# cvxpy/cvxpylayers

Measured on NVIDIA H100. Metric: QP problems/sec fwd+bwd (batch=4096, n=100, m=200, zero+nonneg cones), higher is better.
Workload: dtype f64

## Files before the change

cvxpylayers_b200/csrc/common.cuh:

```cuda
#pragma once
#include <cuda_runtime.h>
#include <stdint.h>
#include <stddef.h>
#include "../../include/bcone.h"

#define BC_TAU_FACTOR 10.0
#define BC_ZERO_CONE_FACTOR 1000.0
#define BC_MIN_SCALE 1e-4
#define BC_MAX_SCALE 1e4
#define BC_RESCALE_MIN_ITERS 100
#define BC_EQ_MIN 1e-4
#define BC_EQ_MAX 1e4

enum { BC_CZERO = 0, BC_CNONNEG = 1, BC_CSOC = 2, BC_CPSD = 3 };

struct DevStruct {
  int n, m, nnzA, nnzP;
  int z, l, nq, ns;
  int ep, ed, exp_start;
  int dense;
  int ncones;
  int max_psd;
  const int *A_indptr, *A_indices;
  const int *At_colptr, *At_rowidx, *At_perm;
// ... 384 lines not shown
__device__ __forceinline__ void dmma884(double &d0, double &d1, double a, double b) {
  asm volatile("mma.sync.aligned.m8n8k4.row.col.f64.f64.f64.f64 {%0,%1}, {%2}, {%3}, {%0,%1};" : "+d"(d0), "+d"(d1) : "d"(a), "d"(b));
}

__device__ __forceinline__ double c_mul_sub(double c, double x, double s, double y) { return fma(c, x, -(s * y)); }
__device__ __forceinline__ double c_mul_add(double s, double x, double c, double y) { return fma(s, x, c * y); }

template <bool SQ = false, class Layout, class Epi>
__device__ __forceinline__ void matvec_rows(const double *__restrict__ M, Layout lay, int nrows, int ncols,
                                            const double *x, Epi ep) {
  const int lane = threadIdx.x & 31, warp = threadIdx.x >> 5, nw = blockDim.x >> 5;
  if (ncols <= 128) {
    double xr[4];
#pragma unroll
    for (int k = 0; k < 4; k++) { const int c = lane + 32 * k; xr[k] = c < ncols ? x[c] : 0.0; }
    for (int i0 = warp * 4; i0 < nrows; i0 += nw * 4) {
      int o[4], b[4], e[4];
#pragma unroll
      for (int r = 0; r < 4; r++) {
        const int i = i0 + r; const bool ok = i < nrows;
        o[r] = ok ? lay.base(i) : 0; b[r] = ok ? lay.beg(i) : 0; e[r] = ok ? lay.end(i) : 0;
      }
      double a[4] = {0, 0, 0, 0};
#pragma unroll
      for (int k = 0; k < 4; k++) {
        const int c = lane + 32 * k;
#pragma unroll
        for (int r = 0; r < 4; r++)
          if (c >= b[r] && c < e[r]) { const double q = M[o[r] + c]; a[r] = fma(SQ ? q * q : q, xr[k], a[r]); }
      }
      const double k = butterfly4(a[0], a[1], a[2], a[3], lane);
      if ((lane & 7) == 0) {
        const int r = i0 + ((lane >> 4) & 1) * 2 + ((lane >> 3) & 1);
        if (r < nrows) ep(r, k);
      }
    }
  } else {
    for (int i0 = warp * 4; i0 < nrows; i0 += nw * 4) {
      int o[4], b[4], e[4];
      int lmax = 0, bmin = 1 << 30;
#pragma unroll
      for (int r = 0; r < 4; r++) {
        const int i = i0 + r; const bool ok = i < nrows;
        o[r] = ok ? lay.base(i) : 0; b[r] = ok ? lay.beg(i) : 0; e[r] = ok ? lay.end(i) : 0;
        lmax = max(lmax, e[r]); if (ok) bmin = min(bmin, b[r]);
      }
      double a[4] = {0, 0, 0, 0};
      for (int c = (min(bmin, lmax) & ~31) + lane; c < lmax; c += 32) {
        const double xv = x[c];
#pragma unroll
        for (int r = 0; r < 4; r++)
          if (c >= b[r] && c < e[r]) { const double q = M[o[r] + c]; a[r] = fma(SQ ? q * q : q, xv, a[r]); }
      }
      const double k = butterfly4(a[0], a[1], a[2], a[3], lane);
      if ((lane & 7) == 0) {
        const int r = i0 + ((lane >> 4) & 1) * 2 + ((lane >> 3) & 1);
        if (r < nrows) ep(r, k);
      }
    }
  }
}

struct ColPlan {
  int j, lo, hi, CH;
  bool active, fits;
};
__device__ __forceinline__ ColPlan make_colplan(int nrows, int ncols) {
  ColPlan p;
  const int T = blockDim.x, t = threadIdx.x;
  p.fits = ncols <= T;
  p.CH = p.fits ? T / ncols : 1;
  p.j = p.fits ? t % ncols : t;
  const int c = p.fits ? t / ncols : 0;
  p.active = p.fits && c < p.CH;
  p.lo = (c * nrows) / p.CH;
  p.hi = ((c + 1) * nrows) / p.CH;
  return p;
}

template <bool SQ = false, class Layout, class Epi>
__device__ __forceinline__ void matvec_cols(const double *__restrict__ M, Layout lay, int nrows, int ncols,
                                            const double *y, double *part, Epi ep, const ColPlan &pl) {
  const int T = blockDim.x, t = threadIdx.x;
  if (pl.fits) {
    if (pl.active) {
      const int j = pl.j;
      int i = max(pl.lo, lay.row_lo(j));
      const int hi = min(pl.hi, lay.row_hi(j, nrows));
      double a0 = 0, a1 = 0;
      if (i < hi) {
        const double *p = M + lay.base(i) + j;
        if (Layout::kFullRows) {
          const int st = lay.step(0);
          for (; i + 3 < hi; i += 4) {
            const double q0 = p[0], q1 = p[st], q2 = p[2 * st], q3 = p[3 * st];
            a0 = fma(SQ ? q0 * q0 : q0, y[i], a0); a1 = fma(SQ ? q1 * q1 : q1, y[i + 1], a1);
            a0 = fma(SQ ? q2 * q2 : q2, y[i + 2], a0); a1 = fma(SQ ? q3 * q3 : q3, y[i + 3], a1);
            p += 4 * st;
          }
          for (; i < hi; i++) { const double q = p[0]; a0 = fma(SQ ? q * q : q, y[i], a0); p += st; }
        } else {
          for (; i + 1 < hi; i += 2) {
            const int s0 = lay.step(i);
            const double q0 = p[0], q1 = p[s0];
            a0 = fma(SQ ? q0 * q0 : q0, y[i], a0); a1 = fma(SQ ? q1 * q1 : q1, y[i + 1], a1);
            p += s0 + lay.step(i + 1);
          }
          if (i < hi) { const double q = p[0]; a0 = fma(SQ ? q * q : q, y[i], a0); }
        }
      }
      part[t] = a0 + a1;
    }
    __syncthreads();
    if (t < ncols) {
      double a = 0;
      for (int cc = 0; cc < pl.CH; cc++) a += part[cc * ncols + t];
      ep(t, a);
    }
    __syncthreads();
  } else {
    for (int j = t; j < ncols; j += T) {
      double a = 0;
      const int hi = lay.row_hi(j, nrows);
      for (int i = lay.row_lo(j); i < hi; i++) { const double q = M[lay.base(i) + j]; a = fma(SQ ? q * q : q, y[i], a); }
      ep(j, a);
    }
    __syncthreads();
  }
}

template <bool SQ = false, class Epi>
__device__ __forceinline__ void dense_rows2(const double *__restrict__ A, int m, int n, const double *x, Epi ep) {
  const int lane = threadIdx.x & 31, warp = threadIdx.x >> 5, nw = blockDim.x >> 5;
  const bool ok0 = 2 * lane < n, ok1 = 2 * lane + 64 < n;
  const double2 x0 = ok0 ? make_double2(x[2 * lane], x[2 * lane + 1]) : make_double2(0.0, 0.0);
  const double2 x1 = ok1 ? make_double2(x[2 * lane + 64], x[2 * lane + 65]) : make_double2(0.0, 0.0);
  for (int i0 = warp * 4; i0 < m; i0 += nw * 4) {
    double a[4] = {0, 0, 0, 0};
#pragma unroll
    for (int r = 0; r < 4; r++) {
      const int i = i0 + r;
      if (i < m) {
        const double2 *p2 = reinterpret_cast<const double2 *>(A + i * n) + lane;
        if (ok0) { double2 q = p2[0]; if (SQ) { q.x *= q.x; q.y *= q.y; } a[r] = fma(q.x, x0.x, a[r]); a[r] = fma(q.y, x0.y, a[r]); }
        if (ok1) { double2 q = p2[32]; if (SQ) { q.x *= q.x; q.y *= q.y; } a[r] = fma(q.x, x1.x, a[r]); a[r] = fma(q.y, x1.y, a[r]); }
      }
    }
    const double tot = butterfly4(a[0], a[1], a[2], a[3], lane);
    if ((lane & 7) == 0) {
      const int i = i0 + ((lane >> 4) & 1) * 2 + ((lane >> 3) & 1);
      if (i < m) ep(i, tot);
    }
  }
}
template <bool SQ = false, class Epi>
__device__ __forceinline__ void dense_cols2(const double *__restrict__ A, int m, int n, const double *y, double *part, Epi ep) {
  const int T = blockDim.x, t = threadIdx.x, npair = n >> 1;
  const int CH = min(8, T / npair), pr = t % npair, c = t / npair;
  if (c < CH) {
    const int lo = (c * m) / CH, hi = ((c + 1) * m) / CH;
    const double2 *p2 = reinterpret_cast<const double2 *>(A + lo * n) + pr;
    double2 a0 = make_double2(0.0, 0.0), a1 = make_double2(0.0, 0.0);
    int i = lo;
    for (; i + 1 < hi; i += 2) {
      double2 q0 = p2[0], q1 = p2[npair];
      if (SQ) { q0.x *= q0.x; q0.y *= q0.y; q1.x *= q1.x; q1.y *= q1.y; }
      const double y0 = y[i], y1 = y[i + 1];
      a0.x = fma(q0.x, y0, a0.x); a0.y = fma(q0.y, y0, a0.y);
      a1.x = fma(q1.x, y1, a1.x); a1.y = fma(q1.y, y1, a1.y);
      p2 += 2 * npair;
    }
    if (i < hi) { double2 q0 = p2[0]; if (SQ) { q0.x *= q0.x; q0.y *= q0.y; } const double y0 = y[i]; a0.x = fma(q0.x, y0, a0.x); a0.y = fma(q0.y, y0, a0.y); }
    *reinterpret_cast<double2 *>(part + c * n + 2 * pr) = make_double2(a0.x + a1.x, a0.y + a1.y);
  }
  __syncthreads();
  if (t < n) {
    double a = 0;
    for (int cc = 0; cc < CH; cc++) a += part[cc * n + t];
    ep(t, a);
  }
  __syncthreads();
}

template <bool SQ = false, class Epi>
__device__ __forceinline__ void csr_rows(const double *__restrict__ vals, const int *__restrict__ indptr,
                                         const int *__restrict__ indices, int nrows,
                                         const double *x, Epi ep) {
  constexpr int G = 4;
  const int g = threadIdx.x % G, grp = threadIdx.x / G, ngrp = blockDim.x / G;
  for (int base = 0; base < nrows; base += ngrp) {
    const int i = base + grp;
    double a = 0;
    if (i < nrows) {
      const int e = __ldg(indptr + i + 1);
      for (int k = __ldg(indptr + i) + g; k < e; k += G) { const double q = vals[k]; a = fma(SQ ? q * q : q, x[__ldg(indices + k)], a); }
    }
    a += __shfl_xor_sync(0xffffffffu, a, 1);
    a += __shfl_xor_sync(0xffffffffu, a, 2);
    if (g == 0 && i < nrows) ep(i, a);
  }
}
template <bool SQ = false, class Epi>
__device__ __forceinline__ void csr_cols(const double *__restrict__ vals, const int *__restrict__ colptr,
                                         const int *__restrict__ rowidx, const int *__restrict__ perm, int ncols,
                                         const double *y, Epi ep) {
  constexpr int G = 4;
  const int g = threadIdx.x % G, grp = threadIdx.x / G, ngrp = blockDim.x / G;
  for (int base = 0; base < ncols; base += ngrp) {
    const int j = base + grp;
    double a = 0;
    if (j < ncols) {
      const int e = __ldg(colptr + j + 1);
      for (int k = __ldg(colptr + j) + g; k < e; k += G) { const double q = vals[__ldg(perm + k)]; a = fma(SQ ? q * q : q, y[__ldg(rowidx + k)], a); }
    }
    a += __shfl_xor_sync(0xffffffffu, a, 1);
    a += __shfl_xor_sync(0xffffffffu, a, 2);
    if (g == 0 && j < ncols) ep(j, a);
  }
}

template <bool DENSE, bool SQ = false, class Epi>
__device__ __forceinline__ void A_mul(const DevStruct &S, const double *Av, const double *x, Epi ep, bool wide = false) {
  if (DENSE && wide) dense_rows2<SQ>(Av, S.m, S.n, x, ep);
  else if (DENSE) matvec_rows<SQ>(Av, DenseLayout{S.n}, S.m, S.n, x, ep);
  else csr_rows<SQ>(Av, S.A_indptr, S.A_indices, S.m, x, ep);
}
template <bool DENSE, bool SQ = false, class Epi>
__device__ __forceinline__ void AT_mul(const DevStruct &S, const double *Av, const double *y, double *part, Epi ep, const ColPlan &plA,
                                       bool wide = false) {
  if (DENSE && wide) dense_cols2<SQ>(Av, S.m, S.n, y, part, ep);
  else if (DENSE) matvec_cols<SQ>(Av, DenseLayout{S.n}, S.m, S.n, y, part, ep, plA);
  else { csr_cols<SQ>(Av, S.At_colptr, S.At_rowidx, S.At_perm, S.n, y, ep); __syncthreads(); }
}

template <bool SQ = false, class Epi>
__device__ __forceinline__ void P_mul(const DevStruct &S, const double *Pv, const double *x, double *part, Epi ep, const ColPlan &plN) {
  const int n = S.n;
  if (S.p_dense) {
    matvec_rows<SQ>(Pv, PackedUpperLayout<false>{n}, n, n, x, ep);
    __syncthreads();
    matvec_cols<SQ>(Pv, PackedUpperLayout<true>{n}, n, n, x, part, ep, plN);
  } else {
    csr_rows<SQ>(Pv, S.P_indptr, S.P_indices, n, x, ep);
    __syncthreads();
    constexpr int G = 4;
    const int g = threadIdx.x % G, grp = threadIdx.x / G, ngrp = blockDim.x / G;
    for (int base = 0; base < n; base += ngrp) {
      const int j = base + grp;
      double a = 0;
      if (j < n) {
        const int e = __ldg(S.Pt_colptr + j + 1);
        for (int k = __ldg(S.Pt_colptr + j) + g; k < e; k += G) {
          const int i = __ldg(S.Pt_rowidx + k);
          if (i != j) { const double q = Pv[__ldg(S.Pt_perm + k)]; a = fma(SQ ? q * q : q, x[i], a); }
        }
      }
      a += __shfl_xor_sync(0xffffffffu, a, 1);
      a += __shfl_xor_sync(0xffffffffu, a, 2);
      if (g == 0 && j < n) ep(j, a);
    }
    __syncthreads();
  }
}

__host__ __device__ __forceinline__ int chol_held_cols(int threads) { return 8 * (threads > 32 ? (threads >> 5) - 1 : 1); }
__host__ __device__ __forceinline__ int chol_scratch_doubles(int n, int threads) {
  const int ld = 8 * ((n + 7) >> 3) - chol_held_cols(threads);
  return 8 * (ld > 0 ? ld : 0) + 2;
}
__device__ __forceinline__ double rsqrt_nr(double x) {
  double y;
  asm("rsqrt.approx.ftz.f64 %0, %1;" : "=d"(y) : "d"(x));
  double e = fma(-x * y, y, 1.0);
  y = fma(0.5 * y, e, y);
  e = fma(-x * y, y, 1.0);
  return fma(0.5 * y, e, y);
}
struct Tri4 { double l00, l10, l11, l20, l21, l22, l30, l31, l32, l33, m00, m10, m11, m20, m21, m22, m30, m31, m32, m33; bool pd; };
__device__ __forceinline__ Tri4 tri4_block(const double *K, int r0, int jb) {
  Tri4 q;
  const double *R0 = K + ((r0 * (r0 + 1)) >> 1) + r0;
  const double *R1 = K + (((r0 + 1) * (r0 + 2)) >> 1) + r0, *R2 = K + (((r0 + 2) * (r0 + 3)) >> 1) + r0, *R3 = K + (((r0 + 3) * (r0 + 4)) >> 1) + r0;
  const double d00 = R0[0];
  const double d10 = jb > 1 ? R1[0] : 0.0, d11 = jb > 1 ? R1[1] : 1.0;
  const double d20 = jb > 2 ? R2[0] : 0.0, d21 = jb > 2 ? R2[1] : 0.0, d22 = jb > 2 ? R2[2] : 1.0;
  const double d30 = jb > 3 ? R3[0] : 0.0, d31 = jb > 3 ? R3[1] : 0.0, d32 = jb > 3 ? R3[2] : 0.0, d33 = jb > 3 ? R3[3] : 1.0;
  const double p0 = d00, r0_ = rsqrt_nr(p0);
  q.l00 = p0 * r0_; q.l10 = d10 * r0_; q.l20 = d20 * r0_; q.l30 = d30 * r0_;
  const double p1 = fma(-q.l10, q.l10, d11), r1_ = rsqrt_nr(p1);
  q.l11 = p1 * r1_; q.l21 = fma(-q.l20, q.l10, d21) * r1_; q.l31 = fma(-q.l30, q.l10, d31) * r1_;
  const double p2 = fma(-q.l21, q.l21, fma(-q.l20, q.l20, d22)), r2_ = rsqrt_nr(p2);
  q.l22 = p2 * r2_; q.l32 = fma(-q.l31, q.l21, fma(-q.l30, q.l20, d32)) * r2_;
  const double p3 = fma(-q.l32, q.l32, fma(-q.l31, q.l31, fma(-q.l30, q.l30, d33))), r3_ = rsqrt_nr(p3);
  q.l33 = p3 * r3_;
  q.pd = (p0 > 0) && (p1 > 0) && (p2 > 0) && (p3 > 0);
  q.m00 = r0_; q.m11 = r1_; q.m22 = r2_; q.m33 = r3_;
  q.m10 = -q.l10 * q.m00 * r1_;
  q.m20 = -fma(q.l21, q.m10, q.l20 * q.m00) * r2_; q.m21 = -q.l21 * q.m11 * r2_;
  q.m30 = -fma(q.l32, q.m20, fma(q.l31, q.m10, q.l30 * q.m00)) * r3_;
  q.m31 = -fma(q.l32, q.m21, q.l31 * q.m11) * r3_; q.m32 = -q.l32 * q.m22 * r3_;
  return q;
}
#ifdef BC_CHOLPROF
#define CP_STAMP(k) if (prof && t == 0) { const long long now_ = clock64(); atomicAdd(prof + (k), (unsigned long long)(now_ - tt)); tt = now_; }
#else
#define CP_STAMP(k)
#endif
static __device__ __noinline__ bool chol_inv_packed(double *K, int n, double *tmp, unsigned long long *prof = nullptr) {
  const int T = blockDim.x, t = threadIdx.x, lane = t & 31, warp = t >> 5, nw = T >> 5;
  const int W = nw > 1 ? nw - 1 : 1, w0 = nw > 1 ? warp - 1 : 0, held = chol_held_cols(T);
  const int lds = max(0, 8 * ((n + 7) >> 3) - held);
  double *Tst = tmp, *flag = tmp + 8 * lds;
  double h0 = 0.0, h1 = 0.0;
  long long t0 = 0;
  if (prof && t == 0) t0 = clock64();
#ifdef BC_CHOLPROF
  long long tt = t0;
#endif
  const int fr = lane >> 2, fc = lane & 3;
  auto rowp = [&](int i) { return K + ((i * (i + 1)) >> 1); };
  auto put_m = [&](int r0, int jb, const Tri4 &q) {
    double *D0 = rowp(r0) + r0;
    D0[0] = q.m00;
    if (jb > 1) { double *D1 = rowp(r0 + 1) + r0; D1[0] = q.m10; D1[1] = q.m11; }
    if (jb > 2) { double *D2 = rowp(r0 + 2) + r0; D2[0] = q.m20; D2[1] = q.m21; D2[2] = q.m22; }
    if (jb > 3) { double *D3 = rowp(r0 + 3) + r0; D3[0] = q.m30; D3[1] = q.m31; D3[2] = q.m32; D3[3] = q.m33; }
  };
  auto diag_block = [&](int J0) {
    const int jb = min(8, n - J0), jb2 = jb - 4;
    const Tri4 a = tri4_block(K, J0, min(4, jb));
    bool pd = a.pd;
    __syncwarp();
    if (lane == 0) put_m(J0, min(4, jb), a);
    if (jb2 > 0) {
      const int r = fr, c = fc;
      const bool own = lane < 16 && r < jb2;
      double *Rr = rowp(J0 + 4 + r) + J0;
      __syncwarp();
      double v = 0.0;
      if (own) {
#pragma unroll
        for (int k = 0; k < 4; k++)
          if (k <= c) v = fma(Rr[k], rowp(J0 + c)[J0 + k], v);
      }
      __syncwarp();
      if (own) Rr[c] = v;
      __syncwarp();
      if (own && c <= r) {
        const double *Rc = rowp(J0 + 4 + c) + J0;
        double g = Rr[4 + c];
#pragma unroll
        for (int k = 0; k < 4; k++) g = fma(-Rr[k], Rc[k], g);
        Rr[4 + c] = g;
      }
      __syncwarp();
      const Tri4 b = tri4_block(K, J0 + 4, jb2);
      pd = pd && b.pd;
      double u = 0.0;
      if (own) {
#pragma unroll
        for (int k = 0; k < 4; k++)
          if (k >= c) u = fma(Rr[k], rowp(J0 + k)[J0 + c], u);
      }
      __syncwarp();
      if (lane == 0) put_m(J0 + 4, jb2, b);
      __syncwarp();
      double s = 0.0;
#pragma unroll
      for (int k = 0; k < 4; k++) {
        const double uk = __shfl_sync(0xffffffffu, u, 4 * k + c);
        if (own && k <= r) s = fma(Rr[4 + k], uk, s);
      }
      if (own) Rr[c] = -s;
    }
    if (lane == 0 && !pd) *flag = 0.0;
  };
  auto trail_tile = [&](int ta, int tb, int J0, int jb, int R0) {
    const int ra = R0 + 8 * ta + fr, rb = R0 + 8 * tb + fr;
    const double *La = rowp(ra) + J0, *Lb = rowp(rb) + J0;
    const double fa0 = (ra < n && fc < jb) ? -La[fc] : 0.0, fa1 = (ra < n && fc + 4 < jb) ? -La[fc + 4] : 0.0;
    const double fb0 = (rb < n && fc < jb) ? Lb[fc] : 0.0, fb1 = (rb < n && fc + 4 < jb) ? Lb[fc + 4] : 0.0;
    const int cc = R0 + 8 * tb + 2 * fc;
    double *pc = rowp(ra) + cc;
    const bool ok0 = ra < n && cc <= ra, ok1 = ra < n && cc + 1 <= ra;
    double c0 = ok0 ? pc[0] : 0.0, c1 = ok1 ? pc[1] : 0.0;
    dmma884(c0, c1, fa0, fb0);
    dmma884(c0, c1, fa1, fb1);
    if (ok0) pc[0] = c0;
    if (ok1) pc[1] = c1;
  };
  auto inv_tile = [&](int jt, int I0, int ib) {
    double c0 = 0.0, c1 = 0.0, d0 = 0.0, d1 = 0.0;
    const bool zr = fr < ib;
    const double *zrow = rowp(I0 + (zr ? fr : 0));
    const int jcol = 8 * jt + fr;
    int k0 = 8 * jt + fc;
    {
      const double a0 = zr ? zrow[k0] : 0.0, a1 = zr ? zrow[k0 + 4] : 0.0;
      const double b0 = jcol <= k0 ? rowp(k0)[jcol] : 0.0, b1 = jcol <= k0 + 4 ? rowp(k0 + 4)[jcol] : 0.0;
      dmma884(c0, c1, a0, b0);
      dmma884(d0, d1, a1, b1);
      k0 += 8;
    }
    int o0 = ((k0 * (k0 + 1)) >> 1) + jcol;
    for (; k0 < I0; k0 += 8) {
      const int o1 = o0 + 4 * k0 + 10;
      const double a0 = zr ? zrow[k0] : 0.0, a1 = zr ? zrow[k0 + 4] : 0.0;
      const double b0 = K[o0], b1 = K[o1];
      dmma884(c0, c1, a0, b0);
      dmma884(d0, d1, a1, b1);
      o0 += 8 * k0 + 36;
    }
    if (jt < W) { h0 = c0 + d0; h1 = c1 + d1; }
    else {
      const int col = 8 * jt + 2 * fc - held;
      Tst[fr * lds + col] = c0 + d0; Tst[fr * lds + col + 1] = c1 + d1;
    }
  };
  auto store_X = [&](int I0) {
    const int ib = min(8, n - I0);
    if ((warp > 0 || nw == 1) && 8 * w0 < I0 && fr < ib) { double *p = rowp(I0 + fr) + 8 * w0 + 2 * fc; p[0] = h0; p[1] = h1; }
    for (int j = held + (t + (T >> 1)) % T; j < I0; j += T) {
#pragma unroll
      for (int r = 0; r < 8; r++)
        if (r < ib) rowp(I0 + r)[j] = Tst[r * lds + j - held];
    }
  };
  if (warp == 0) {
    if (lane == 0) *flag = 1.0;
    __syncwarp();
    diag_block(0);
  }
  __syncthreads();
  for (int J0 = 0; J0 < n; J0 += 8) {
    const int jb = min(8, n - J0), R0 = J0 + jb;
    if (*flag == 0.0) return false;
    if (J0 > 0) store_X(J0 - 8);
    const int tz = (t + T - (T >> 2)) % T;
    if (R0 + t < n || tz < J0) {
      const double *Md = rowp(J0) + J0;
      for (int i = R0 + t; i < n; i += T) {
        double *row = rowp(i) + J0;
        double a[8];
#pragma unroll
        for (int c = 0; c < 8; c++) a[c] = c < jb ? row[c] : 0.0;
#pragma unroll
        for (int c = 0; c < 8; c++) {
          if (c < jb) {
            const double *Mc = Md + ((c * (c + 1)) >> 1) + c * J0;
            double s = 0.0;
#pragma unroll
            for (int k = 0; k <= c; k++) s = fma(a[k], Mc[k], s);
            row[c] = s;
          }
        }
      }
      for (int i = tz; i < J0; i += T) {
        double a[8];
#pragma unroll
        for (int r = 0; r < 8; r++) a[r] = r < jb ? rowp(J0 + r)[i] : 0.0;
#pragma unroll
        for (int r = 0; r < 8; r++) {
          if (r < jb) {
            const double *Mr = Md + ((r * (r + 1)) >> 1) + r * J0;
            double s = 0.0;
#pragma unroll
            for (int k = 0; k <= r; k++) s = fma(Mr[k], a[k], s);
            rowp(J0 + r)[i] = -s;
          }
        }
      }
    }
    CP_STAMP(17);
    __syncthreads();
    CP_STAMP(18);
    {
      const int ntl = R0 < n ? (n - R0 + 7) >> 3 : 0, ntile = (ntl * (ntl + 1)) >> 1;
      const int ntj = J0 >> 3;
      if (warp == 0 && ntile > 0) {
        trail_tile(0, 0, J0, jb, R0);
        __syncwarp();
        diag_block(R0);
      }
      if (warp > 0 || nw == 1) {
        const int nwork = ntj + (ntile > 0 ? ntile - 1 : 0);
        int ta = 0, tb = 0, e_cur = 0;
        for (int u = w0; u < nwork; u += W) {
          if (u < ntj) inv_tile(u, J0, jb);
          else {
            const int e = u - ntj + 1;
            tb += e - e_cur; e_cur = e;
            while (tb > ta) { tb -= ta + 1; ta++; }
            trail_tile(ta, tb, J0, jb, R0);
          }
        }
      }
    }
    CP_STAMP(19);
    __syncthreads();
    CP_STAMP(20);
  }
  if (*flag == 0.0) return false;
  store_X(((n - 1) >> 3) << 3);
  __syncthreads();
  if (prof && t == 0) { const long long t1 = clock64(); atomicAdd(prof + 5, (unsigned long long)(t1 - t0)); }
  return true;
}

__device__ void jacobi_eig_warp(int k, double *X, double *V);

__device__ __forceinline__ void project_soc_warp(double *v, int sz) {
  const int lane = threadIdx.x & 31;
  if (sz == 1) { if (lane == 0 && v[0] < 0) v[0] = 0; return; }
  double ss = 0;
  for (int i = 1 + lane; i < sz; i += 32) ss += v[i] * v[i];
  ss = warp_sum(ss);
  const double nx = sqrt(ss), t = v[0];
  __syncwarp();
  if (nx <= t) return;
  if (nx <= -t) { for (int i = lane; i < sz; i += 32) v[i] = 0; return; }
  const double a = 0.5 * (1.0 + t / nx);
  for (int i = 1 + lane; i < sz; i += 32) v[i] *= a;
  if (lane == 0) v[0] = a * nx;
}

__device__ __forceinline__ void svec_to_mat_warp(int k, const double *v, double *X) {
  const int lane = threadIdx.x & 31;
  const double is2 = 0.70710678118654752440;
  for (int e = lane; e < k * k; e += 32) {
    int i = e / k, j = e % k;
    int r = max(i, j), c = min(i, j);
    int idx = c * k - (c * (c - 1)) / 2 + (r - c);
    X[e] = (i == j) ? v[idx] : v[idx] * is2;
  }
}
__device__ __forceinline__ void mat_to_svec_warp(int k, const double *X, double *v) {
  const int lane = threadIdx.x & 31;
  const double s2 = 1.41421356237309504880;
  for (int e = lane; e < k * k; e += 32) {
    int i = e / k, j = e % k;
    if (i < j) continue;
    int idx = j * k - (j * (j - 1)) / 2 + (i - j);
    v[idx] = (i == j) ? X[i * k + i] : 0.5 * (X[i * k + j] + X[j * k + i]) * s2;
  }
}

__device__ inline void jacobi_eig_warp(int k, double *X, double *V) {
  const int lane = threadIdx.x & 31;
  for (int e = lane; e < k * k; e += 32) V[e] = (e / k == e % k) ? 1.0 : 0.0;
  __syncwarp();
  for (int sweep = 0; sweep < 30; sweep++) {
    int rotations = 0;
    for (int p = 0; p < k - 1; p++) for (int q = p + 1; q < k; q++) {
      const double apq = X[p * k + q];
      if (fabs(apq) <= 1e-17 * (fabs(X[p * k + p]) + fabs(X[q * k + q])) || apq == 0.0) continue;
      rotations++;
      const double app = X[p * k + p], aqq = X[q * k + q];
      const double theta = (aqq - app) / (2.0 * apq);
      const double t = (theta >= 0 ? 1.0 : -1.0) / (fabs(theta) + sqrt(theta * theta + 1.0));
      const double c = 1.0 / sqrt(t * t + 1.0), s = t * c;
      __syncwarp();
      for (int r = lane; r < k; r += 32) {
        double xp = X[r * k + p], xq = X[r * k + q];
        X[r * k + p] = c * xp - s * xq; X[r * k + q] = s * xp + c * xq;
        double vp = V[r * k + p], vq = V[r * k + q];
        V[r * k + p] = c * vp - s * vq; V[r * k + q] = s * vp + c * vq;
      }
      __syncwarp();
      for (int r = lane; r < k; r += 32) {
        double xp = X[p * k + r], xq = X[q * k + r];
        X[p * k + r] = c * xp - s * xq; X[q * k + r] = s * xp + c * xq;
      }
      __syncwarp();
    }
    if (rotations == 0) break;
  }
  __syncwarp();
}

template <class FA, class FB, class ST>
__device__ __forceinline__ void warp_mm16(int k, FA fa, FB fb, ST st) {
  const int lane = threadIdx.x & 31, fr = lane >> 2, fc = lane & 3;
  const int nt = (k + 7) >> 3, nk = (k + 3) >> 2;
  for (int ti = 0; ti < nt; ti++) {
    double d[2][2] = {{0.0, 0.0}, {0.0, 0.0}};
    for (int ks = 0; ks < nk; ks++) {
      const double a = fa(8 * ti + fr, 4 * ks + fc);
#pragma unroll
      for (int tj = 0; tj < 2; tj++) if (tj < nt) dmma884(d[tj][0], d[tj][1], a, fb(4 * ks + fc, 8 * tj + fr));
    }
#pragma unroll
    for (int tj = 0; tj < 2; tj++) if (tj < nt) { st(8 * ti + fr, 8 * tj + 2 * fc, d[tj][0]); st(8 * ti + fr, 8 * tj + 2 * fc + 1, d[tj][1]); }
  }
}

__device__ __forceinline__ double rcp_nr(double x) {
  double y;
  asm("rcp.approx.ftz.f64 %0, %1;" : "=d"(y) : "d"(x));
  double e = fma(-x, y, 1.0);
  y = fma(y, e, y);
  e = fma(-x, y, 1.0);
  return fma(y, e, y);
}
__device__ inline void jacobi_par_warp(int k, double *T, double *V) {
  const int lane = threadIdx.x & 31;
  const int kk = (k + 1) & ~1, np = kk >> 1, nr = kk - 1;
  constexpr int MAXT = 4;
  int ln[MAXT], pj_[MAXT];
  const int ntrip = (k * np + 31) >> 5;
#pragma unroll
  for (int tr = 0; tr < MAXT; tr++) { const int e = lane + 32 * tr; ln[tr] = e < k * np ? e / np : -1; pj_[tr] = e < k * np ? e - (e / np) * np : 0; }
  auto pair_of = [&](int r, int j, int &p, int &q) {
    int a = r + j; if (a >= nr) a -= nr;
    int b = r - j; if (b < 0) b += nr;
    if (j == 0) { a = kk - 1; b = r; }
    p = min(a, b); q = max(a, b);
  };
  for (int sweep = 0; sweep < 30; sweep++) {
    bool big = false;
    for (int r = 0; r < nr; r++) {
      double c = 1.0, s = 0.0;
      if (lane < np) {
        int p, q;
        pair_of(r, lane, p, q);
        if (q < k) {
          const double apq = T[p * k + q], app = T[p * k + p], aqq = T[q * k + q];
          const double lim = fabs(app) + fabs(aqq);
          if (!(fabs(apq) <= 1e-17 * lim) && apq != 0.0) {
            big = big || fabs(apq) > 1e-7 * lim;
            const double theta = (aqq - app) * rcp_nr(2.0 * apq), th2 = fma(theta, theta, 1.0);
            const double t = (theta >= 0 ? 1.0 : -1.0) * rcp_nr(fabs(theta) + th2 * rsqrt_nr(th2));
            c = rsqrt_nr(fma(t, t, 1.0)); s = t * c;
          }
        }
      }
      __syncwarp();
#pragma unroll
      for (int tr = 0; tr < MAXT; tr++) {
        if (tr < ntrip) {
          const double cj = __shfl_sync(0xffffffffu, c, pj_[tr]), sj = __shfl_sync(0xffffffffu, s, pj_[tr]);
          int p, q;
          pair_of(r, pj_[tr], p, q);
          if (ln[tr] >= 0 && q < k && sj != 0.0) {
            const int row = ln[tr];
            const double xp = T[row * k + p], xq = T[row * k + q];
            T[row * k + p] = c_mul_sub(cj, xp, sj, xq); T[row * k + q] = c_mul_add(sj, xp, cj, xq);
            const double vp = V[row * k + p], vq = V[row * k + q];
            V[row * k + p] = c_mul_sub(cj, vp, sj, vq); V[row * k + q] = c_mul_add(sj, vp, cj, vq);
          }
        }
      }
      __syncwarp();
#pragma unroll
      for (int tr = 0; tr < MAXT; tr++) {
        if (tr < ntrip) {
          const double cj = __shfl_sync(0xffffffffu, c, pj_[tr]), sj = __shfl_sync(0xffffffffu, s, pj_[tr]);
          int p, q;
          pair_of(r, pj_[tr], p, q);
          if (ln[tr] >= 0 && q < k && sj != 0.0) {
            const int col = ln[tr];
            const double xp = T[p * k + col], xq = T[q * k + col];
            T[p * k + col] = c_mul_sub(cj, xp, sj, xq); T[q * k + col] = c_mul_add(sj, xp, cj, xq);
          }
        }
      }
      __syncwarp();
    }
    if (!__any_sync(0xffffffffu, big)) break;
  }
}

__device__ inline void project_psd_warp(double *v, int k, double *scr, double *Vp = nullptr, bool warm = false) {
  const int lane = threadIdx.x & 31;
  double *X = scr, *W = scr + k * k, *lam = W + k * k;
  svec_to_mat_warp(k, v, X);
  __syncwarp();
  if (k > 16 || !Vp) {
    jacobi_eig_warp(k, X, W);
    for (int i = lane; i < k; i += 32) lam[i] = fmax(X[i * k + i], 0.0);
    __syncwarp();
    for (int e = lane; e < k * k; e += 32) {
      int i = e / k, j = e % k;
      double a = 0;
      for (int q = 0; q < k; q++) a = fma(W[i * k + q] * lam[q], W[j * k + q], a);
      X[e] = a;
    }
    __syncwarp();
    mat_to_svec_warp(k, X, v);
    __syncwarp();
    return;
  }
  auto inb = [&](int i, int j) { return i < k && j < k; };
  if (warm) {
    warp_mm16(k, [&](int i, int q) { return inb(i, q) ? X[i * k + q] : 0.0; }, [&](int q, int j) { return inb(q, j) ? Vp[q * k + j] : 0.0; },
              [&](int i, int j, double val) { if (inb(i, j)) W[i * k + j] = val; });
    __syncwarp();
    warp_mm16(k, [&](int i, int q) { return inb(i, q) ? Vp[q * k + i] : 0.0; }, [&](int q, int j) { return inb(q, j) ? W[q * k + j] : 0.0; },
              [&](int i, int j, double val) { if (inb(i, j)) X[i * k + j] = val; });
    __syncwarp();
  } else {
    for (int e = lane; e < k * k; e += 32) Vp[e] = (e / k == e % k) ? 1.0 : 0.0;
    __syncwarp();
  }
  jacobi_par_warp(k, X, Vp);
  for (int i = lane; i < k; i += 32) lam[i] = fmax(X[i * k + i], 0.0);
  __syncwarp();
  warp_mm16(k, [&](int i, int q) { return inb(i, q) ? Vp[i * k + q] * lam[q] : 0.0; }, [&](int q, int j) { return inb(q, j) ? Vp[j * k + q] : 0.0; },
            [&](int i, int j, double val) { if (inb(i, j)) W[i * k + j] = val; });
  __syncwarp();
  mat_to_svec_warp(k, W, v);
  __syncwarp();
}

__device__ inline double exp_newton_one_d(double rho, double yh, double zh) {
  double t = fmax(-zh, 1e-6);
  for (int i = 0; i < 100; i++) {
    const double f = t * (t + zh) / rho / rho - yh / rho + log(t / rho) + 1.0;
    const double fp = (2.0 * t + zh) / rho / rho + 1.0 / t;
    t -= f / fp;
    if (t <= -zh) return 0.0;
    if (t <= 0.0) return zh;
    if (fabs(f) < 1e-13) break;
  }
  return t + zh;
}
__device__ inline double exp_calc_grad(const double *v, double *x, double rho) {
  x[2] = exp_newton_one_d(rho, v[1], v[2]);
  x[1] = (x[2] - v[2]) * x[2] / rho;
  x[0] = v[0] - rho;
  if (x[1] <= 1e-12) return x[0];
  return x[0] + x[1] * log(x[1] / x[2]);
}
__device__ inline double exp_h(double r, double s, double t, double rho, double *y, double *mu) {
  const double E = exp(rho), id = 1.0 / (rho + E * E);
  *y = (r + t * E) * id;
  *mu = (r * E - t * rho) * id;
  return *y + *mu * E * (1.0 - rho) - s;
}
__device__ inline bool exp_newton_rho(double r, double s, double t, double *rho0, double *x) {
  double rho = (rho0 && *rho0 == *rho0) ? *rho0 : (s > 0 ? fmin(fmax(r / s, -20.0), 20.0) : (t > 0 && r > 0 ? fmin(log(fmax(t, 1e-300) / fmax(r, 1e-300)) , 20.0) : 0.0));
  const double scale = fmax(1.0, fmax(fabs(r), fmax(fabs(s), fabs(t))));
  double y, mu, hv = exp_h(r, s, t, rho, &y, &mu);
  for (int it = 0; it < 30; it++) {
    if (!(hv == hv)) return false;
    if (fabs(hv) <= 1e-15 * scale) break;
    const double E = exp(rho), den = rho + E * E;
    const double yp = (t * E * den - (r + t * E) * (1.0 + 2.0 * E * E)) / (den * den);
    const double mup = (yp + y) * E;
    const double hp = yp + mup * E * (1.0 - rho) - mu * E * rho;
    if (hp == 0.0 || !(hp == hp)) return false;
    double step = -hv / hp, rn, yn, mn, hn;
    int bt = 0;
    bool stalled = false;
    for (;; bt++) {
      rn = rho + step;
      hn = exp_h(r, s, t, rn, &yn, &mn);
      if (hn == hn && fabs(hn) < fabs(hv)) break;
      if (bt == 12) { stalled = true; break; }
      step *= 0.5;
    }
    if (stalled) {
      if (fabs(hv) <= 1e-11 * scale) break;
      return false;
    }
    const bool tiny = fabs(step) <= 1e-15 * fmax(1.0, fabs(rn));
    rho = rn; hv = hn; y = yn; mu = mn;
    if (tiny) break;
  }
  if (!(fabs(hv) <= 1e-11 * scale) || !(y > 0)) return false;
  const double E = exp(rho);
  const double px = y * rho, py = y, pz = y * E;
  const double dx = r - px, dy = s - py, dz = t - pz;
  const double na = E >= 1.0 ? 1.0 : E, n0 = na, n1 = na * (1.0 - rho), n2 = E >= 1.0 ? -1.0 / E : -1.0;
  const double nn = sqrt(n0 * n0 + n1 * n1 + n2 * n2), mu2 = (dx * n0 + dy * n1 + dz * n2) / nn;
  if (!(mu2 >= -1e-13 * scale)) return false;
  if (fabs(dx - mu2 * n0 / nn) > 1e-9 * scale || fabs(dy - mu2 * n1 / nn) > 1e-9 * scale || fabs(dz - mu2 * n2 / nn) > 1e-9 * scale) return false;
  if (fabs(px * dx + py * dy + pz * dz) > 1e-9 * scale * scale) return false;
  x[0] = px; x[1] = py; x[2] = pz;
  if (rho0) *rho0 = rho;
  return true;
}
__device__ inline bool exp_newton_multi(double r, double s, double t, double *rho0, double *x) {
  if (exp_newton_rho(r, s, t, rho0, x)) return true;
  const double starts[6] = {0.0, -1.0, 1.0, -3.0, 3.0, 8.0};
#pragma unroll 1
  for (int k = 0; k < 6; k++) {
    double g = starts[k];
    if (exp_newton_rho(r, s, t, &g, x)) { if (rho0) *rho0 = g; return true; }
  }
  return false;
}
__device__ inline int proj_exp_unit(double *v, double *rho0) {
  const double r = v[0], s = v[1], t = v[2];
  if ((s > 0 && s * exp(fmin(r / s, 700.0)) - t <= 1e-13) || (r <= 0 && s == 0 && t >= 0)) return 0;
  if ((r > 0 && r * exp(fmin(s / r, 700.0)) + 2.718281828459045 * t <= 1e-13) || (r == 0 && s <= 0 && t <= 0)) { v[0] = v[1] = v[2] = 0; return 1; }
  if (r < 0 && s < 0) { v[1] = 0.0; v[2] = fmax(t, 0.0); return 2; }
  double x[3];
  if (exp_newton_multi(r, s, t, rho0, x)) { v[0] = x[0]; v[1] = x[1]; v[2] = x[2]; return 3; }
  if (rho0) *rho0 = nan("");
  double lb = 0.0, ub = 0.125;
  while (exp_calc_grad(v, x, ub) > 0 && ub < 1e300) { lb = ub; ub *= 2.0; }
  for (int i = 0; i < 200; i++) {
    const double rho = 0.5 * (ub + lb), g = exp_calc_grad(v, x, rho);
    if (g > 0) lb = rho; else ub = rho;
    if (ub - lb < 1e-10 * fmax(1.0, rho)) break;
  }
// ... 249 lines not shown
```

Baseline: 252,900.

## Overlap Cholesky diagonal-block factorization with worker panel updates via named barrier

Restructures the blocked packed Cholesky-inverse so warp 0 computes the first panel row-block and then immediately does the next diagonal-block trailing update and factorization, signalling worker warps through a named barrier (bar.arrive/bar.sync 1) rather than a full __syncthreads. Worker warps do the remaining panel rows, the store of the previous inverse rows, and the inverse and trailing tiles, with the trailing tile loads batched two at a time to raise memory-level parallelism. One block-wide barrier per column step is removed. The failure flag is double-buffered so the early diagonal factorization does not race with the current step's check. The cost is more complex synchronization and a risk of subtle races.

```diff
diff --git a/cvxpylayers_b200/csrc/common.cuh b/cvxpylayers_b200/csrc/common.cuh
--- a/cvxpylayers_b200/csrc/common.cuh
+++ b/cvxpylayers_b200/csrc/common.cuh
@@ -710,23 +710,30 @@
   return q;
 }
 #ifdef BC_CHOLPROF
-#define CP_STAMP(k) if (prof && t == 0) { const long long now_ = clock64(); atomicAdd(prof + (k), (unsigned long long)(now_ - tt)); tt = now_; }
+#define CP_MARK(who) if (prof && t == (who)) tt = clock64();
+#define CP_STAMP(k, who) if (prof && t == (who)) { const long long now_ = clock64(); atomicAdd(prof + (k), (unsigned long long)(now_ - tt)); tt = now_; }
 #else
-#define CP_STAMP(k)
+#define CP_MARK(who)
+#define CP_STAMP(k, who)
 #endif
 static __device__ __noinline__ bool chol_inv_packed(double *K, int n, double *tmp, unsigned long long *prof = nullptr) {
   const int T = blockDim.x, t = threadIdx.x, lane = t & 31, warp = t >> 5, nw = T >> 5;
   const int W = nw > 1 ? nw - 1 : 1, w0 = nw > 1 ? warp - 1 : 0, held = chol_held_cols(T);
+  const int Tw = 32 * W, tw = t - (T - Tw);
+  const bool worker = warp > 0 || nw == 1;
   const int lds = max(0, 8 * ((n + 7) >> 3) - held);
   double *Tst = tmp, *flag = tmp + 8 * lds;
   double h0 = 0.0, h1 = 0.0;
   long long t0 = 0;
   if (prof && t == 0) t0 = clock64();
 #ifdef BC_CHOLPROF
-  long long tt = t0;
+  long long tt = clock64();
+  const int tw0 = T - Tw;
 #endif
   const int fr = lane >> 2, fc = lane & 3;
   auto rowp = [&](int i) { return K + ((i * (i + 1)) >> 1); };
+  auto nb_sync = [&] { asm volatile("bar.sync 1, %0;" : : "r"(nw > 1 ? T : 32) : "memory"); };
+  auto nb_arrive = [&] { asm volatile("bar.arrive 1, %0;" : : "r"(T) : "memory"); };
   auto put_m = [&](int r0, int jb, const Tri4 &q) {
     double *D0 = rowp(r0) + r0;
     D0[0] = q.m00;
@@ -781,21 +788,34 @@
       }
       if (own) Rr[c] = -s;
     }
-    if (lane == 0 && !pd) *flag = 0.0;
+    if (lane == 0 && !pd) flag[(J0 >> 3) & 1] = 0.0;
   };
-  auto trail_tile = [&](int ta, int tb, int J0, int jb, int R0) {
+  auto panel_entry = [&](const double *a, const double *Md, int J0, int c) {
+    const double *Mc = Md + ((c * (c + 1)) >> 1) + c * J0;
+    double s = 0.0;
+#pragma unroll
+    for (int k = 0; k < 8; k++)
+      if (k <= c) s = fma(a[k], Mc[k], s);
+    return s;
+  };
+  struct Trail { double fa0, fa1, fb0, fb1, c0, c1; double *pc; bool ok0, ok1; };
+  auto trail_load = [&](int ta, int tb, int J0, int jb, int R0) {
+    Trail q;
     const int ra = R0 + 8 * ta + fr, rb = R0 + 8 * tb + fr;
     const double *La = rowp(ra) + J0, *Lb = rowp(rb) + J0;
-    const double fa0 = (ra < n && fc < jb) ? -La[fc] : 0.0, fa1 = (ra < n && fc + 4 < jb) ? -La[fc + 4] : 0.0;
-    const double fb0 = (rb < n && fc < jb) ? Lb[fc] : 0.0, fb1 = (rb < n && fc + 4 < jb) ? Lb[fc + 4] : 0.0;
+    q.fa0 = (ra < n && fc < jb) ? -La[fc] : 0.0; q.fa1 = (ra < n && fc + 4 < jb) ? -La[fc + 4] : 0.0;
+    q.fb0 = (rb < n && fc < jb) ? Lb[fc] : 0.0; q.fb1 = (rb < n && fc + 4 < jb) ? Lb[fc + 4] : 0.0;
     const int cc = R0 + 8 * tb + 2 * fc;
-    double *pc = rowp(ra) + cc;
-    const bool ok0 = ra < n && cc <= ra, ok1 = ra < n && cc + 1 <= ra;
-    double c0 = ok0 ? pc[0] : 0.0, c1 = ok1 ? pc[1] : 0.0;
-    dmma884(c0, c1, fa0, fb0);
-    dmma884(c0, c1, fa1, fb1);
-    if (ok0) pc[0] = c0;
-    if (ok1) pc[1] = c1;
+    q.pc = rowp(ra) + cc;
+    q.ok0 = ra < n && cc <= ra; q.ok1 = ra < n && cc + 1 <= ra;
+    q.c0 = q.ok0 ? q.pc[0] : 0.0; q.c1 = q.ok1 ? q.pc[1] : 0.0;
+    return q;
+  };
+  auto trail_store = [&](Trail &q) {
+    dmma884(q.c0, q.c1, q.fa0, q.fb0);
+    dmma884(q.c0, q.c1, q.fa1, q.fb1);
+    if (q.ok0) q.pc[0] = q.c0;
+    if (q.ok1) q.pc[1] = q.c1;
   };
   auto inv_tile = [&](int jt, int I0, int ib) {
     double c0 = 0.0, c1 = 0.0, d0 = 0.0, d1 = 0.0;
@@ -827,43 +847,62 @@
   };
   auto store_X = [&](int I0) {
     const int ib = min(8, n - I0);
-    if ((warp > 0 || nw == 1) && 8 * w0 < I0 && fr < ib) { double *p = rowp(I0 + fr) + 8 * w0 + 2 * fc; p[0] = h0; p[1] = h1; }
-    for (int j = held + (t + (T >> 1)) % T; j < I0; j += T) {
+    if (8 * w0 < I0 && fr < ib) { double *p = rowp(I0 + fr) + 8 * w0 + 2 * fc; p[0] = h0; p[1] = h1; }
+    for (int j = held + (tw + Tw - 32 * (W >> 1)) % Tw; j < I0; j += Tw) {
 #pragma unroll
       for (int r = 0; r < 8; r++)
         if (r < ib) rowp(I0 + r)[j] = Tst[r * lds + j - held];
     }
   };
   if (warp == 0) {
-    if (lane == 0) *flag = 1.0;
+    if (lane == 0) flag[0] = flag[1] = 1.0;
     __syncwarp();
     diag_block(0);
   }
   __syncthreads();
   for (int J0 = 0; J0 < n; J0 += 8) {
     const int jb = min(8, n - J0), R0 = J0 + jb;
-    if (*flag == 0.0) return false;
-    if (J0 > 0) store_X(J0 - 8);
-    const int tz = (t + T - (T >> 2)) % T;
-    if (R0 + t < n || tz < J0) {
-      const double *Md = rowp(J0) + J0;
-      for (int i = R0 + t; i < n; i += T) {
+    if (flag[(J0 >> 3) & 1] == 0.0) return false;
+    const double *Md = rowp(J0) + J0;
+    const int ntl = R0 < n ? (n - R0 + 7) >> 3 : 0, ntile = (ntl * (ntl + 1)) >> 1;
+    if (warp == 0) {
+      CP_MARK(0);
+      const int i = R0 + fr;
+      double *row = rowp(i) + J0;
+      double v0 = 0.0, v1 = 0.0;
+      if (i < n) {
+        double a[8];
+#pragma unroll
+        for (int c = 0; c < 8; c++) a[c] = c < jb ? row[c] : 0.0;
+        v0 = panel_entry(a, Md, J0, fc); v1 = panel_entry(a, Md, J0, 7 - fc);
+      }
+      __syncwarp();
+      if (i < n) {
+        if (fc < jb) row[fc] = v0;
+        if (7 - fc < jb) row[7 - fc] = v1;
+      }
+      __syncwarp();
+      if (nw > 1) nb_arrive();
+      if (ntile > 0) {
+        Trail q = trail_load(0, 0, J0, jb, R0);
+        trail_store(q);
+        __syncwarp();
+        diag_block(R0);
+      }
+      CP_STAMP(21, 0);
+    }
+    if (worker) {
+      if (J0 > 0) store_X(J0 - 8);
+      for (int i = R0 + 8 + tw; i < n; i += Tw) {
         double *row = rowp(i) + J0;
         double a[8];
 #pragma unroll
         for (int c = 0; c < 8; c++) a[c] = c < jb ? row[c] : 0.0;
 #pragma unroll
-        for (int c = 0; c < 8; c++) {
-          if (c < jb) {
-            const double *Mc = Md + ((c * (c + 1)) >> 1) + c * J0;
-            double s = 0.0;
-#pragma unroll
-            for (int k = 0; k <= c; k++) s = fma(a[k], Mc[k], s);
-            row[c] = s;
-          }
-        }
-      }
-      for (int i = tz; i < J0; i += T) {
+        for (int c = 0; c < 8; c++)
+          if (c < jb) row[c] = panel_entry(a, Md, J0, c);
+      }
+      for (int i = (tw + Tw - 32 * (W >> 2)) % Tw; i < J0; i += Tw) {
         double a[8];
 #pragma unroll
         for (int r = 0; r < 8; r++) a[r] = r < jb ? rowp(J0 + r)[i] : 0.0;
@@ -878,38 +917,37 @@
           }
         }
       }
-    }
-    CP_STAMP(17);
+      CP_STAMP(17, tw0);
+      nb_sync();
+      CP_STAMP(18, tw0);
+      const int ntj = J0 >> 3;
+      const int nwork = ntj + (ntile > 0 ? ntile - 1 : 0);
+      int u = w0;
+      for (; u < ntj; u += W) inv_tile(u, J0, jb);
+      int ta = 0, tb = 0, e_cur = 0;
+      auto next_tile = [&](int v) {
+        const int e = v - ntj + 1;
+        tb += e - e_cur; e_cur = e;
+        while (tb > ta) { tb -= ta + 1; ta++; }
+      };
+      for (; u < nwork; u += 2 * W) {
+        next_tile(u);
+        Trail q0 = trail_load(ta, tb, J0, jb, R0);
+        if (u + W < nwork) {
+          next_tile(u + W);
+          Trail q1 = trail_load(ta, tb, J0, jb, R0);
+          trail_store(q0);
+          trail_store(q1);
+        } else {
+          trail_store(q0);
+        }
+      }
+      CP_STAMP(19, tw0);
+    }
     __syncthreads();
-    CP_STAMP(18);
-    {
-      const int ntl = R0 < n ? (n - R0 + 7) >> 3 : 0, ntile = (ntl * (ntl + 1)) >> 1;
-      const int ntj = J0 >> 3;
-      if (warp == 0 && ntile > 0) {
-        trail_tile(0, 0, J0, jb, R0);
-        __syncwarp();
-        diag_block(R0);
-      }
-      if (warp > 0 || nw == 1) {
-        const int nwork = ntj + (ntile > 0 ? ntile - 1 : 0);
-        int ta = 0, tb = 0, e_cur = 0;
-        for (int u = w0; u < nwork; u += W) {
-          if (u < ntj) inv_tile(u, J0, jb);
-          else {
-            const int e = u - ntj + 1;
-            tb += e - e_cur; e_cur = e;
-            while (tb > ta) { tb -= ta + 1; ta++; }
-            trail_tile(ta, tb, J0, jb, R0);
-          }
-        }
-      }
-    }
-    CP_STAMP(19);
-    __syncthreads();
-    CP_STAMP(20);
-  }
-  if (*flag == 0.0) return false;
-  store_X(((n - 1) >> 3) << 3);
+    CP_STAMP(20, tw0);
+  }
+  if (worker) store_X(((n - 1) >> 3) << 3);
   __syncthreads();
   if (prof && t == 0) { const long long t1 = clock64(); atomicAdd(prof + 5, (unsigned long long)(t1 - t0)); }
   return true;
```

Result: faster. 255,900, median of 6 (+1.2%).
